# PaddlePaddle/Parakeet

Hardware: NVIDIA H100
Metric: audio-samples/sec (higher is better)
Workload: dtype bf16x3 (split-bf16 operands, fp32 accumulate; fp32-grade, 1e-3 parity)

## Files before the change

### parakeet_b200/csrc/pk_common.cu

```cuda
#include <stdarg.h>
#include <stdio.h>
#include <string.h>

#include <atomic>

#include "pk_host.h"

namespace pk {

static thread_local char g_err[512] = "";
static std::atomic<long long> g_launches{0};

void set_error(const char* fmt, ...) {
  va_list ap;
  va_start(ap, fmt);
  vsnprintf(g_err, sizeof(g_err), fmt, ap);
  va_end(ap);
}

int fail(int code, const char* fmt, ...) {
  va_list ap;
  va_start(ap, fmt);
  vsnprintf(g_err, sizeof(g_err), fmt, ap);
  va_end(ap);
  return code;
}

void count_launch(int n) { g_launches.fetch_add(n, std::memory_order_relaxed); }

int sm_count() {
  static std::atomic<int> cache[64];
  int dev = 0;
  if (cudaGetDevice(&dev) != cudaSuccess || dev < 0 || dev >= 64) return 132;
  int n = cache[dev].load(std::memory_order_relaxed);
  if (n == 0) {
    if (cudaDeviceGetAttribute(&n, cudaDevAttrMultiProcessorCount, dev) != cudaSuccess || n <= 0) n = 132;
    cache[dev].store(n, std::memory_order_relaxed);
  }
  return n;
}

typedef CUresult (*EncodeTiledFn)(CUtensorMap*, CUtensorMapDataType, cuuint32_t, void*, const cuuint64_t*, const cuuint64_t*,
                                  const cuuint32_t*, const cuuint32_t*, CUtensorMapInterleave, CUtensorMapSwizzle,
                                  CUtensorMapL2promotion, CUtensorMapFloatOOBfill);

static EncodeTiledFn get_encode_fn() {
  static EncodeTiledFn fn = nullptr;
  if (fn == nullptr) {
    void* p = nullptr;
    cudaDriverEntryPointQueryResult qres;
    if (cudaGetDriverEntryPoint("cuTensorMapEncodeTiled", &p, cudaEnableDefault, &qres) == cudaSuccess &&
        qres == cudaDriverEntryPointSuccess)
      fn = reinterpret_cast<EncodeTiledFn>(p);
  }
  return fn;
}

int encode_tmap_bf16_3d(CUtensorMap* out, const void* base, uint64_t cols, uint64_t rows, uint64_t batches,
                        uint64_t row_stride_elems, uint64_t batch_stride_elems, uint32_t box_rows) {
  EncodeTiledFn fn = get_encode_fn();
  if (fn == nullptr) return fail(PK_ERR_CUDA, "cuTensorMapEncodeTiled entry point not available (no CUDA driver?)");
  if (batches == 0) batches = 1;
  if (batch_stride_elems == 0) batch_stride_elems = row_stride_elems * rows;
  cuuint64_t dims[3] = {cols, rows, batches};
  cuuint64_t strides[2] = {row_stride_elems * 2, batch_stride_elems * 2};
  cuuint32_t box[3] = {64, box_rows, 1};
  cuuint32_t estr[3] = {1, 1, 1};
  if ((strides[0] & 15) || (strides[1] & 15)) return fail(PK_ERR_INVALID_ARG, "TMA strides must be multiples of 16 bytes");
  CUresult r = fn(out, CU_TENSOR_MAP_DATA_TYPE_BFLOAT16, 3, const_cast<void*>(base), dims, strides, box, estr,
                  CU_TENSOR_MAP_INTERLEAVE_NONE, CU_TENSOR_MAP_SWIZZLE_128B, CU_TENSOR_MAP_L2_PROMOTION_L2_256B,
                  CU_TENSOR_MAP_FLOAT_OOB_FILL_NONE);
  if (r != CUDA_SUCCESS)
    return fail(PK_ERR_CUDA, "cuTensorMapEncodeTiled failed (%d): cols=%llu rows=%llu batches=%llu ld=%llu bs=%llu box_rows=%u",
                static_cast<int>(r), (unsigned long long)cols, (unsigned long long)rows, (unsigned long long)batches,
                (unsigned long long)row_stride_elems, (unsigned long long)batch_stride_elems, box_rows);
  return PK_OK;
}

int encode_tmap_bf16_planes(CUtensorMap* out, const void* hi, const void* lo, uint64_t cols, uint64_t rows, uint64_t batches,
                            uint64_t row_stride_elems, uint64_t batch_stride_elems, uint32_t box_rows, uint32_t box_cols) {
  EncodeTiledFn fn = get_encode_fn();
  if (fn == nullptr) return fail(PK_ERR_CUDA, "cuTensorMapEncodeTiled entry point not available (no CUDA driver?)");
  if (box_cols != 64 && box_cols != 16) return fail(PK_ERR_INVALID_ARG, "box_cols must be 64 or 16 (got %u)", box_cols);
  const CUtensorMapSwizzle swz = box_cols == 64 ? CU_TENSOR_MAP_SWIZZLE_128B : CU_TENSOR_MAP_SWIZZLE_32B;
  const long long plane = static_cast<const char*>(lo) - static_cast<const char*>(hi);
  if (plane <= 0 || (plane & 15) || plane >= (1ll << 40))
    return fail(PK_ERR_INVALID_ARG, "split planes must come from one allocation, lo after hi at a 16-byte multiple (ops.Split.empty / zeros)");
  if (batches == 0) batches = 1;
  if (batch_stride_elems == 0) batch_stride_elems = row_stride_elems * rows;
  cuuint64_t dims[4] = {cols, rows, batches, 2};
  cuuint64_t strides[3] = {row_stride_elems * 2, batch_stride_elems * 2, static_cast<cuuint64_t>(plane)};
  cuuint32_t box[4] = {box_cols, box_rows, 1, 2};
  cuuint32_t estr[4] = {1, 1, 1, 1};
  if ((strides[0] & 15) || (strides[1] & 15)) return fail(PK_ERR_INVALID_ARG, "TMA strides must be multiples of 16 bytes");
  CUresult r = fn(out, CU_TENSOR_MAP_DATA_TYPE_BFLOAT16, 4, const_cast<void*>(hi), dims, strides, box, estr,
                  CU_TENSOR_MAP_INTERLEAVE_NONE, swz, CU_TENSOR_MAP_L2_PROMOTION_L2_256B,
                  CU_TENSOR_MAP_FLOAT_OOB_FILL_NONE);
  if (r != CUDA_SUCCESS)
    return fail(PK_ERR_CUDA, "cuTensorMapEncodeTiled (4-D planes) failed (%d): cols=%llu rows=%llu batches=%llu ld=%llu bs=%llu plane=%lld",
                static_cast<int>(r), (unsigned long long)cols, (unsigned long long)rows, (unsigned long long)batches,
                (unsigned long long)row_stride_elems, (unsigned long long)batch_stride_elems, plane);
  return PK_OK;
}

}

extern "C" int pk_version(void) { return 100;  }
extern "C" const char* pk_last_error(void) { return pk::g_err; }
extern "C" int64_t pk_launch_count(void) { return pk::g_launches.load(std::memory_order_relaxed); }
```

### parakeet_b200/csrc/pk_host.h

```cpp
#pragma once
#include <cuda.h>
#include <cuda_runtime.h>
#include <stdint.h>

#include "../../include/parakeet_b200.h"

namespace pk {

void set_error(const char* fmt, ...);
int fail(int code, const char* fmt, ...);

#define PK_CHECK_ARG(cond, ...)                                   \
  do {                                                            \
    if (!(cond)) return ::pk::fail(PK_ERR_INVALID_ARG, __VA_ARGS__); \
  } while (0)

#define PK_CHECK_CUDA(expr)                                                                          \
  do {                                                                                               \
    cudaError_t _e = (expr);                                                                         \
    if (_e != cudaSuccess) return ::pk::fail(PK_ERR_CUDA, "%s: %s", #expr, cudaGetErrorString(_e)); \
  } while (0)

int encode_tmap_bf16_3d(CUtensorMap* out, const void* base, uint64_t cols, uint64_t rows, uint64_t batches,
                        uint64_t row_stride_elems, uint64_t batch_stride_elems, uint32_t box_rows);

int encode_tmap_bf16_planes(CUtensorMap* out, const void* hi, const void* lo, uint64_t cols, uint64_t rows, uint64_t batches,
                            uint64_t row_stride_elems, uint64_t batch_stride_elems, uint32_t box_rows, uint32_t box_cols = 64);

int sm_count();
void count_launch(int n = 1);

}
```

### parakeet_b200/csrc/pk_sm90.cuh

```cuda
#pragma once
#include <cuda.h>
#include <cuda_bf16.h>
#include <cuda_runtime.h>
#include <stdint.h>

namespace pk {

constexpr int kSwizzleBytes = 128;
constexpr int kChunkK = 64;

__device__ __forceinline__ uint32_t smem_u32(const void* p) {
  return static_cast<uint32_t>(__cvta_generic_to_shared(p));
}

__device__ __forceinline__ void fence_barrier_init() {
  asm volatile("fence.mbarrier_init.release.cluster;" ::: "memory");
}

__device__ __forceinline__ void fence_proxy_async_all() { asm volatile("fence.proxy.async;" ::: "memory"); }
__device__ __forceinline__ void fence_proxy_async_shared() { asm volatile("fence.proxy.async.shared::cta;" ::: "memory"); }

__device__ __forceinline__ void tma_prefetch_desc(const CUtensorMap* tm) {
  asm volatile("prefetch.tensormap [%0];" ::"l"(reinterpret_cast<uint64_t>(tm)) : "memory");
}

constexpr int kWgmmaK = 16;

__device__ __forceinline__ uint64_t make_smem_desc_sw128(uint32_t smem_addr) {
  uint64_t d = 0;
  d |= static_cast<uint64_t>((smem_addr & 0x3FFFFu) >> 4);
  d |= static_cast<uint64_t>(1) << 16;
  d |= static_cast<uint64_t>(1024 >> 4) << 32;
  d |= static_cast<uint64_t>(1) << 62;
  return d;
}
__device__ __forceinline__ uint64_t desc_kstep(int k) { return static_cast<uint64_t>((k * kWgmmaK * 2) >> 4); }
__device__ __forceinline__ uint64_t make_smem_desc_sw32(uint32_t smem_addr) {
  uint64_t d = 0;
  d |= static_cast<uint64_t>((smem_addr & 0x3FFFFu) >> 4);
  d |= static_cast<uint64_t>(1) << 16;
  d |= static_cast<uint64_t>(256 >> 4) << 32;
  d |= static_cast<uint64_t>(3) << 62;
  return d;
}

__device__ __forceinline__ void wgmma_fence() { asm volatile("wgmma.fence.sync.aligned;" ::: "memory"); }
__device__ __forceinline__ void wgmma_commit() { asm volatile("wgmma.commit_group.sync.aligned;" ::: "memory"); }
template <int N>
__device__ __forceinline__ void wgmma_wait() { asm volatile("wgmma.wait_group.sync.aligned %0;" ::"n"(N) : "memory"); }
template <int R>
__device__ __forceinline__ void reg_fence(float (&d)[R]) {
#pragma unroll
  for (int i = 0; i < R; ++i) asm volatile("" : "+f"(d[i])::"memory");
}
template <uint32_t kRegs>
__device__ __forceinline__ void setmaxnreg_dec() { asm volatile("setmaxnreg.dec.sync.aligned.u32 %0;" ::"n"(kRegs)); }
template <uint32_t kRegs>
__device__ __forceinline__ void setmaxnreg_inc() { asm volatile("setmaxnreg.inc.sync.aligned.u32 %0;" ::"n"(kRegs)); }
__device__ __forceinline__ void named_bar_sync(int id, int threads) {
  asm volatile("bar.sync %0, %1;" ::"r"(id), "r"(threads) : "memory");
}
__device__ __forceinline__ void named_bar_arrive(int id, int threads) {
  asm volatile("bar.arrive %0, %1;" ::"r"(id), "r"(threads) : "memory");
}

#define PK_F8(i) "+f"(d[i]), "+f"(d[i + 1]), "+f"(d[i + 2]), "+f"(d[i + 3]), "+f"(d[i + 4]), "+f"(d[i + 5]), "+f"(d[i + 6]), "+f"(d[i + 7])
#define PK_F32(i) PK_F8(i), PK_F8(i + 8), PK_F8(i + 16), PK_F8(i + 24)
#define PK_D32 "%0,%1,%2,%3,%4,%5,%6,%7,%8,%9,%10,%11,%12,%13,%14,%15,%16,%17,%18,%19,%20,%21,%22,%23,%24,%25,%26,%27,%28,%29,%30,%31"
#define PK_D64 PK_D32 ",%32,%33,%34,%35,%36,%37,%38,%39,%40,%41,%42,%43,%44,%45,%46,%47,%48,%49,%50,%51,%52,%53,%54,%55,%56,%57,%58,%59,%60,%61,%62,%63"
#define PK_D96 PK_D64 ",%64,%65,%66,%67,%68,%69,%70,%71,%72,%73,%74,%75,%76,%77,%78,%79,%80,%81,%82,%83,%84,%85,%86,%87,%88,%89,%90,%91,%92,%93,%94,%95"
#define PK_D128 PK_D96 ",%96,%97,%98,%99,%100,%101,%102,%103,%104,%105,%106,%107,%108,%109,%110,%111,%112,%113,%114,%115,%116,%117,%118,%119,%120,%121,%122,%123,%124,%125,%126,%127"
__device__ __forceinline__ void wgmma_ss_n64(float (&d)[32], uint64_t adesc, uint64_t bdesc, uint32_t accumulate) {
  asm volatile("{\n.reg .pred p;\nsetp.ne.b32 p, %34, 0;\n"
               "wgmma.mma_async.sync.aligned.m64n64k16.f32.bf16.bf16 {" PK_D32 "}, %32, %33, p, 1, 1, 0, 0;\n}\n"
               : PK_F32(0) : "l"(adesc), "l"(bdesc), "r"(accumulate));
}
__device__ __forceinline__ void wgmma_ss_n128(float (&d)[64], uint64_t adesc, uint64_t bdesc, uint32_t accumulate) {
  asm volatile("{\n.reg .pred p;\nsetp.ne.b32 p, %66, 0;\n"
               "wgmma.mma_async.sync.aligned.m64n128k16.f32.bf16.bf16 {" PK_D64 "}, %64, %65, p, 1, 1, 0, 0;\n}\n"
               : PK_F32(0), PK_F32(32) : "l"(adesc), "l"(bdesc), "r"(accumulate));
}
__device__ __forceinline__ void wgmma_ss_n256(float (&d)[128], uint64_t adesc, uint64_t bdesc, uint32_t accumulate) {
  asm volatile("{\n.reg .pred p;\nsetp.ne.b32 p, %130, 0;\n"
               "wgmma.mma_async.sync.aligned.m64n256k16.f32.bf16.bf16 {" PK_D128 "}, %128, %129, p, 1, 1, 0, 0;\n}\n"
               : PK_F32(0), PK_F32(32), PK_F32(64), PK_F32(96) : "l"(adesc), "l"(bdesc), "r"(accumulate));
}
__device__ __forceinline__ void wgmma_rs_n64(float (&d)[32], const uint32_t (&a)[4], uint64_t bdesc, uint32_t accumulate) {
  asm volatile("{\n.reg .pred p;\nsetp.ne.b32 p, %37, 0;\n"
               "wgmma.mma_async.sync.aligned.m64n64k16.f32.bf16.bf16 {" PK_D32 "}, {%32,%33,%34,%35}, %36, p, 1, 1, 0;\n}\n"
               : PK_F32(0) : "r"(a[0]), "r"(a[1]), "r"(a[2]), "r"(a[3]), "l"(bdesc), "r"(accumulate));
}
__device__ __forceinline__ void wgmma_rs_n128(float (&d)[64], const uint32_t (&a)[4], uint64_t bdesc, uint32_t accumulate) {
  asm volatile("{\n.reg .pred p;\nsetp.ne.b32 p, %69, 0;\n"
               "wgmma.mma_async.sync.aligned.m64n128k16.f32.bf16.bf16 {" PK_D64 "}, {%64,%65,%66,%67}, %68, p, 1, 1, 0;\n}\n"
               : PK_F32(0), PK_F32(32) : "r"(a[0]), "r"(a[1]), "r"(a[2]), "r"(a[3]), "l"(bdesc), "r"(accumulate));
}
__device__ __forceinline__ void wgmma_rs_n192(float (&d)[96], const uint32_t (&a)[4], uint64_t bdesc, uint32_t accumulate) {
  asm volatile("{\n.reg .pred p;\nsetp.ne.b32 p, %101, 0;\n"
               "wgmma.mma_async.sync.aligned.m64n192k16.f32.bf16.bf16 {" PK_D96 "}, {%96,%97,%98,%99}, %100, p, 1, 1, 0;\n}\n"
               : PK_F32(0), PK_F32(32), PK_F32(64) : "r"(a[0]), "r"(a[1]), "r"(a[2]), "r"(a[3]), "l"(bdesc), "r"(accumulate));
}
#undef PK_F32
#undef PK_F8

__device__ __forceinline__ void philox4x32_10(uint32_t c0, uint32_t c1, uint32_t c2, uint32_t c3, uint32_t k0, uint32_t k1, uint32_t* out) {
#pragma unroll
  for (int r = 0; r < 10; ++r) {
    const uint32_t hi0 = __umulhi(0xD2511F53u, c0), lo0 = 0xD2511F53u * c0;
    const uint32_t hi1 = __umulhi(0xCD9E8D57u, c2), lo1 = 0xCD9E8D57u * c2;
    c0 = hi1 ^ c1 ^ k0; c1 = lo1; c2 = hi0 ^ c3 ^ k1; c3 = lo0;
    k0 += 0x9E3779B9u; k1 += 0xBB67AE85u;
  }
  out[0] = c0; out[1] = c1; out[2] = c2; out[3] = c3;
}

__device__ __forceinline__ void split_bf16(float v, __nv_bfloat16& hi, __nv_bfloat16& lo) {
  hi = __float2bfloat16_rn(v);
  lo = __float2bfloat16_rn(v - __bfloat162float(hi));
}
__device__ __forceinline__ uint32_t pack_bf16x2(__nv_bfloat16 a, __nv_bfloat16 b) {
  return static_cast<uint32_t>(__bfloat16_as_ushort(a)) | (static_cast<uint32_t>(__bfloat16_as_ushort(b)) << 16);
}
__device__ __forceinline__ void split8(const float* v, uint4& hi, uint4& lo) {
  __nv_bfloat16 h[8], l[8];
#pragma unroll
  for (int i = 0; i < 8; ++i) split_bf16(v[i], h[i], l[i]);
  hi = make_uint4(pack_bf16x2(h[0], h[1]), pack_bf16x2(h[2], h[3]), pack_bf16x2(h[4], h[5]), pack_bf16x2(h[6], h[7]));
  lo = make_uint4(pack_bf16x2(l[0], l[1]), pack_bf16x2(l[2], l[3]), pack_bf16x2(l[4], l[5]), pack_bf16x2(l[6], l[7]));
}


__device__ __forceinline__ float4 lds_f4(uint32_t addr) {
  float4 v;
  asm volatile("ld.shared.v4.f32 {%0, %1, %2, %3}, [%4];" : "=f"(v.x), "=f"(v.y), "=f"(v.z), "=f"(v.w) : "r"(addr));
  return v;
}
__device__ __forceinline__ uint32_t lds_u32(uint32_t addr) {
  uint32_t v;
  asm volatile("ld.shared.u32 %0, [%1];" : "=r"(v) : "r"(addr) : "memory");
  return v;
}
__device__ __forceinline__ void sts_u32(uint32_t addr, uint32_t v) {
  asm volatile("st.shared.u32 [%0], %1;" ::"r"(addr), "r"(v) : "memory");
}

__device__ __forceinline__ void mbar_init_a(uint32_t bar, uint32_t count) {
  asm volatile("mbarrier.init.shared::cta.b64 [%0], %1;" ::"r"(bar), "r"(count) : "memory");
}
__device__ __forceinline__ void mbar_arrive_expect_tx_a(uint32_t bar, uint32_t bytes) {
  asm volatile("mbarrier.arrive.expect_tx.shared::cta.b64 _, [%0], %1;" ::"r"(bar), "r"(bytes) : "memory");
}
__device__ __forceinline__ void mbar_arrive_a(uint32_t bar) {
  asm volatile("mbarrier.arrive.shared::cta.b64 _, [%0];" ::"r"(bar) : "memory");
}
__device__ __forceinline__ void mbar_wait_a(uint32_t bar, uint32_t parity) {
  uint32_t ok = 0;
  for (uint32_t spin = 0; spin < (1u << 26); ++spin) {
    asm volatile(
        "{\n"
        ".reg .pred p;\n"
        "mbarrier.try_wait.parity.shared::cta.b64 p, [%1], %2;\n"
        "selp.u32 %0, 1, 0, p;\n"
        "}\n"
        : "=r"(ok)
        : "r"(bar), "r"(parity)
        : "memory");
    if (ok) return;
  }
  __trap();
}
__device__ __forceinline__ void tma_load_3d_a(uint32_t smem_dst, const CUtensorMap* tm, uint32_t bar, int c0, int c1, int c2) {
  asm volatile(
      "cp.async.bulk.tensor.3d.shared::cluster.global.tile.mbarrier::complete_tx::bytes [%0], [%1, {%3, %4, %5}], [%2];"
      ::"r"(smem_dst), "l"(reinterpret_cast<uint64_t>(tm)), "r"(bar), "r"(c0), "r"(c1), "r"(c2)
      : "memory");
}
__device__ __forceinline__ void tma_load_4d_a(uint32_t smem_dst, const CUtensorMap* tm, uint32_t bar, int c0, int c1, int c2, int c3) {
  asm volatile(
      "cp.async.bulk.tensor.4d.shared::cluster.global.tile.mbarrier::complete_tx::bytes [%0], [%1, {%3, %4, %5, %6}], [%2];"
      ::"r"(smem_dst), "l"(reinterpret_cast<uint64_t>(tm)), "r"(bar), "r"(c0), "r"(c1), "r"(c2), "r"(c3)
      : "memory");
}
__device__ __forceinline__ void tma_store_4d_a(const CUtensorMap* tm, uint32_t smem_src, int c0, int c1, int c2, int c3) {
  asm volatile("cp.async.bulk.tensor.4d.global.shared::cta.bulk_group [%0, {%2, %3, %4, %5}], [%1];"
               ::"l"(reinterpret_cast<uint64_t>(tm)), "r"(smem_src), "r"(c0), "r"(c1), "r"(c2), "r"(c3)
               : "memory");
}
__device__ __forceinline__ void bulk_prefetch_l2(const void* gptr, uint32_t bytes) {
  asm volatile("cp.async.bulk.prefetch.L2.global [%0], %1;" ::"l"(reinterpret_cast<uint64_t>(gptr)), "r"(bytes) : "memory");
}
__device__ __forceinline__ void bulk_commit() { asm volatile("cp.async.bulk.commit_group;" ::: "memory"); }
template <int N>
__device__ __forceinline__ void bulk_wait_read() { asm volatile("cp.async.bulk.wait_group.read %0;" ::"n"(N) : "memory"); }


constexpr int kStageSlotBytes = 64 * 32 * 4;
__device__ __forceinline__ uint32_t stage_addr(uint32_t slot, int row, int col) {
  return slot + row * 128 + ((((col >> 2) ^ (row & 7)) << 4) | ((col & 3) << 2));
}
template <int R>
__device__ __forceinline__ void stage_store(uint32_t slot, const float (&d)[R], int C, int wg_thread) {
  const int w = wg_thread >> 5, lane = wg_thread & 31;
  const int r0 = 16 * w + (lane >> 2), c0 = 2 * (lane & 3);
#pragma unroll
  for (int jj = 0; jj < 4; ++jj) {
    const int j = 4 * C + jj;
    asm volatile("st.shared.v2.f32 [%0], {%1, %2};" ::"r"(stage_addr(slot, r0, 8 * jj + c0)), "f"(d[4 * j]), "f"(d[4 * j + 1]) : "memory");
    asm volatile("st.shared.v2.f32 [%0], {%1, %2};" ::"r"(stage_addr(slot, r0 + 8, 8 * jj + c0)), "f"(d[4 * j + 2]), "f"(d[4 * j + 3])
                 : "memory");
  }
}
__device__ __forceinline__ void stage_load_row(uint32_t slot, int row, float (&v)[32]) {
#pragma unroll
  for (int k = 0; k < 8; ++k) {
    const float4 x = lds_f4(slot + row * 128 + ((k ^ (row & 7)) << 4));
    v[4 * k] = x.x; v[4 * k + 1] = x.y; v[4 * k + 2] = x.z; v[4 * k + 3] = x.w;
  }
}

}
```

### parakeet_b200/csrc/pwg_fc.cu

```cuda
#include <stdlib.h>
#include <string.h>

#include <algorithm>

#include "pk_host.h"
#include "pk_sm90.cuh"

namespace pk {
namespace fc {

constexpr int kPwgR = 64;
constexpr int kPwgG = 128;
constexpr int kATile = 128 * kSwizzleBytes;
constexpr int kQTile = 64 * kSwizzleBytes;
constexpr int kConsumerThreads = 256;
constexpr int kThreads = kConsumerThreads + 128;
constexpr int kFcG1Chunks = 4;
constexpr int kFcStages = 6;
constexpr int kFcStageBytes = 2 * kQTile;
constexpr int kFcUBytes = 2 * 64 * 32;
constexpr int kFcPBytes = 2 * 128 * 32;
constexpr int kFcW1Bytes = 3 * 2 * kATile;
constexpr int kFcW2Bytes = 2 * kATile;
constexpr int kFcSmem = kFcW1Bytes + kFcW2Bytes + kFcStages * kFcStageBytes + 1024 + 256;
static_assert(kFcUBytes + kFcPBytes <= kFcStageBytes, "the conditioning operands share one ring stage");
static_assert(kFcSmem <= 227 * 1024, "shared memory budget");

struct FcLayerArgs {
  int batch, t, dil, hop;
  int u_period, u_start_row, u_end_base;
  int p_row0;
  const int32_t* lens;
  float gate_c[128];
  float out_b[64];
  float k_a, k_g;
  float* skip;
  int skip_init;
};

__device__ __forceinline__ float ex2_approx(float x) {
  float y;
  asm("ex2.approx.ftz.f32 %0, %1;" : "=f"(y) : "f"(x));
  return y;
}
__device__ __forceinline__ float rcp_approx(float x) {
  float y;
  asm("rcp.approx.ftz.f32 %0, %1;" : "=f"(y) : "f"(x));
  return y;
}
__device__ __forceinline__ void split2(float a, float b, uint32_t& hi, uint32_t& lo) {
  const __nv_bfloat162 h = __floats2bfloat162_rn(a, b);
  hi = *reinterpret_cast<const uint32_t*>(&h);
  const float ra = a - __uint_as_float(hi << 16);
  const float rb = b - __uint_as_float(hi & 0xffff0000u);
  const __nv_bfloat162 l = __floats2bfloat162_rn(ra, rb);
  lo = *reinterpret_cast<const uint32_t*>(&l);
}

struct FcTileIter {
  int idx, step, tiles_per_b, total, t;
  const int32_t* lens;
  __device__ FcTileIter(const FcLayerArgs& p)
      : idx(static_cast<int>(blockIdx.x) - static_cast<int>(gridDim.x)), step(gridDim.x),
        tiles_per_b((p.t + 255) >> 8), total(((p.t + 255) >> 8) * p.batch * 2), t(p.t), lens(p.lens) {}
  __device__ bool next(int& b, int& m0, int& half) {
    for (;;) {
      idx += step;
      if (idx >= total) return false;
      const int w = idx >> 1;
      half = idx & 1;
      b = w / tiles_per_b;
      m0 = (w % tiles_per_b) * 256;
      const int len = lens ? min(__ldg(lens + b), t) : t;
      if (m0 < len) return true;
    }
  }
};

__global__ void __launch_bounds__(kThreads, 1)
pwg_layer_fc_kernel(const __grid_constant__ CUtensorMap tm_x, const __grid_constant__ CUtensorMap tm_u,
                    const __grid_constant__ CUtensorMap tm_p,
                    const __grid_constant__ CUtensorMap tm_w1_hi, const __grid_constant__ CUtensorMap tm_w1_lo,
                    const __grid_constant__ CUtensorMap tm_w2_hi, const __grid_constant__ CUtensorMap tm_w2_lo,
                    const __grid_constant__ CUtensorMap tm_y, const FcLayerArgs p) {
  extern __shared__ uint8_t smem_raw[];
  const uint32_t smem = (smem_u32(smem_raw) + 1023u) & ~1023u;
  const uint32_t w1 = smem;
  const uint32_t w2 = w1 + kFcW1Bytes;
  const uint32_t ring = w2 + kFcW2Bytes;
  const uint32_t bars = ring + kFcStages * kFcStageBytes;
  const uint32_t full_bar = bars;
  const uint32_t empty_bar = full_bar + 8 * kFcStages;
  const uint32_t w_bar = empty_bar + 8 * kFcStages;

  const int warp = threadIdx.x >> 5;
  const int lane = threadIdx.x & 31;

  if (threadIdx.x == kConsumerThreads) {
    tma_prefetch_desc(&tm_x); tma_prefetch_desc(&tm_u); tma_prefetch_desc(&tm_p);
    tma_prefetch_desc(&tm_w1_hi); tma_prefetch_desc(&tm_w1_lo); tma_prefetch_desc(&tm_w2_hi); tma_prefetch_desc(&tm_w2_lo);
    tma_prefetch_desc(&tm_y);
    for (int s = 0; s < kFcStages; ++s) { mbar_init_a(full_bar + 8 * s, 1); mbar_init_a(empty_bar + 8 * s, 4); }
    mbar_init_a(w_bar, 1);
    fence_barrier_init();
  }
  __syncthreads();

  if (warp >= kConsumerThreads / 32) {
    setmaxnreg_dec<40>();
    if (warp == kConsumerThreads / 32 && lane == 0) {
      mbar_arrive_expect_tx_a(w_bar, kFcW1Bytes + kFcW2Bytes);
      for (int j = 0; j < 3; ++j) {
        tma_load_3d_a(w1 + j * 2 * kATile, &tm_w1_hi, w_bar, j * kChunkK, 0, 0);
        tma_load_3d_a(w1 + j * 2 * kATile + kATile, &tm_w1_lo, w_bar, j * kChunkK, 0, 0);
      }
      tma_load_3d_a(w2, &tm_w2_hi, w_bar, 0, 0, 0);
      tma_load_3d_a(w2 + kATile, &tm_w2_lo, w_bar, 0, 0, 0);
      uint32_t it = 0;
      FcTileIter ti(p);
      int b, m0, half;
      while (ti.next(b, m0, half)) {
        const int mh = m0 + 128 * half;
        const int len = p.lens ? min(__ldg(p.lens + b), p.t) : p.t;
        const int m1 = ((len - 128) >> 7) << 7;
        const int urow = mh == 0 ? p.u_start_row
                         : (mh + 128 > len - 128) ? p.u_end_base + 384 * b + min(mh - m1, 256)
                                                  : mh % p.u_period;
        const int j0 = (m0 / p.hop - 2) & ~7;
        for (int wg = 0; wg < 2; ++wg) {
          const int rows = min(64, p.t - (mh + 64 * wg));
          if (!p.skip_init && rows > 0)
            bulk_prefetch_l2(p.skip + (static_cast<long long>(b) * p.t + mh + 64 * wg) * 64, rows * 64 * 4);
          for (int j = 0; j < kFcG1Chunks; ++j, ++it) {
            const int s = it % kFcStages;
            mbar_wait_a(empty_bar + 8 * s, ((it / kFcStages) & 1) ^ 1);
            const uint32_t st = ring + s * kFcStageBytes;
            const uint32_t fb = full_bar + 8 * s;
            if (j == 2) {
              mbar_arrive_expect_tx_a(fb, kFcUBytes + kFcPBytes);
              tma_load_4d_a(st, &tm_u, fb, 0, urow + 64 * wg, 0, 0);
              tma_load_4d_a(st + kFcUBytes, &tm_p, fb, j0, p.p_row0, b, 0);
            } else {
              mbar_arrive_expect_tx_a(fb, kFcStageBytes);
              const int wj = j == 0 ? 0 : j == 1 ? 2 : 1;
              tma_load_4d_a(st, &tm_x, fb, 0, mh + 64 * wg + (wj - 1) * p.dil, b, 0);
            }
          }
        }
      }
    }
  } else {
    setmaxnreg_inc<232>();
    const int wg = warp >> 2;
    const int rl = 16 * (warp & 3) + (lane >> 2);
    const int cq = 2 * (lane & 3);
    const float kSqrtHalf = 0.70710678118654752440f;
    mbar_wait_a(w_bar, 0);
    uint32_t it = wg * kFcG1Chunks;
    FcTileIter ti(p);
    int b, m0, half;
    bool more = ti.next(b, m0, half);
    bool first = true;
    while (more) {
      const int mh = m0 + 128 * half;
      float acc1[64], acc2[64];
      if (wg == 1 || !first) named_bar_sync(1 + wg, kConsumerThreads);
      first = false;
#pragma unroll
      for (int j = 0; j < kFcG1Chunks; ++j) {
        const int s = (it + j) % kFcStages;
        mbar_wait_a(full_bar + 8 * s, ((it + j) / kFcStages) & 1);
        const uint32_t st = ring + s * kFcStageBytes;
        wgmma_fence();
        if (j == 2) {
          const uint64_t a_hi = make_smem_desc_sw32(st), a_lo = make_smem_desc_sw32(st + kFcUBytes / 2);
          const uint64_t b_hi = make_smem_desc_sw32(st + kFcUBytes), b_lo = make_smem_desc_sw32(st + kFcUBytes + kFcPBytes / 2);
          wgmma_ss_n128(acc1, a_hi, b_hi, 1);
          wgmma_ss_n128(acc1, a_lo, b_hi, 1);
          wgmma_ss_n128(acc1, a_hi, b_lo, 1);
        } else {
          const int wj = j == 0 ? 0 : j == 1 ? 2 : 1;
          const uint64_t a_hi = make_smem_desc_sw128(st), a_lo = make_smem_desc_sw128(st + kQTile);
          const uint64_t b_hi = make_smem_desc_sw128(w1 + wj * 2 * kATile), b_lo = make_smem_desc_sw128(w1 + wj * 2 * kATile + kATile);
#pragma unroll
          for (int k = 0; k < 4; ++k) {
            wgmma_ss_n128(acc1, a_hi + desc_kstep(k), b_hi + desc_kstep(k), !(j == 0 && k == 0));
            wgmma_ss_n128(acc1, a_lo + desc_kstep(k), b_hi + desc_kstep(k), 1);
            wgmma_ss_n128(acc1, a_hi + desc_kstep(k), b_lo + desc_kstep(k), 1);
          }
        }
        wgmma_commit();
        if (j == kFcG1Chunks - 1) {
#pragma unroll
          for (int jj = 0; jj < 8; ++jj) {
#pragma unroll
            for (int hh = 0; hh < 2; ++hh) {
              const int r = rl + 8 * hh;
              const uint32_t off = r * kSwizzleBytes + ((((8 * jj + cq) >> 3) ^ (r & 7)) << 4) + (cq & 7) * 2;
              const uint32_t xh = lds_u32(st + off), xl = lds_u32(st + kQTile + off);
              acc2[4 * jj + 2 * hh] = 0.f;
              acc2[4 * jj + 2 * hh + 1] = 0.f;
              acc2[32 + 4 * jj + 2 * hh] = __uint_as_float(xh << 16) + __uint_as_float(xl << 16);
              acc2[32 + 4 * jj + 2 * hh + 1] = __uint_as_float(xh & 0xffff0000u) + __uint_as_float(xl & 0xffff0000u);
            }
          }
        }
        if (j > 0) {
          wgmma_wait<1>();
          __syncwarp();
          if (lane == 0) mbar_arrive_a(empty_bar + 8 * ((it + j - 1) % kFcStages));
        }
      }
      wgmma_wait<0>();
      reg_fence(acc1);
      const int cs = (it + kFcG1Chunks - 1) % kFcStages;
      const uint32_t ystage = ring + cs * kFcStageBytes;
      it += 2 * kFcG1Chunks;
      int nb, nm0, nhalf;
      const bool next = ti.next(nb, nm0, nhalf);
      if (wg == 0 || next) named_bar_arrive(2 - wg, kConsumerThreads);
      uint32_t zh[16], zl[16];
#pragma unroll
      for (int jj = 0; jj < 8; ++jj) {
        float z[4];
#pragma unroll
        for (int e = 0; e < 4; ++e) {
          const int c = 8 * jj + cq + (e & 1);
          const float e1 = ex2_approx(fminf(fmaf(acc1[4 * jj + e], p.k_a, p.gate_c[c]), 60.f));
          const float e2 = ex2_approx(fmaf(acc1[32 + 4 * jj + e], p.k_g, p.gate_c[64 + c]));
          const float t1 = 1.f + e1;
          z[e] = (1.f - e1) * rcp_approx(fmaf(t1, e2, t1));
        }
        split2(z[0], z[1], zh[2 * jj], zl[2 * jj]);
        split2(z[2], z[3], zh[2 * jj + 1], zl[2 * jj + 1]);
      }
      const uint64_t b2_hi = make_smem_desc_sw128(w2), b2_lo = make_smem_desc_sw128(w2 + kATile);
      wgmma_fence();
#pragma unroll
      for (int k = 0; k < 4; ++k) {
        const uint32_t ah[4] = {zh[4 * k], zh[4 * k + 1], zh[4 * k + 2], zh[4 * k + 3]};
        const uint32_t al[4] = {zl[4 * k], zl[4 * k + 1], zl[4 * k + 2], zl[4 * k + 3]};
        wgmma_rs_n128(acc2, ah, b2_hi + desc_kstep(k), 1);
        wgmma_rs_n128(acc2, al, b2_hi + desc_kstep(k), 1);
        wgmma_rs_n128(acc2, ah, b2_lo + desc_kstep(k), 1);
      }
      wgmma_commit();
      wgmma_wait<0>();
      reg_fence(acc2);
      const int len = p.lens ? min(__ldg(p.lens + b), p.t) : p.t;
#pragma unroll
      for (int hh = 0; hh < 2; ++hh) {
        const int r = rl + 8 * hh;
        const bool live = mh + wg * 64 + r < len;
#pragma unroll
        for (int jj = 0; jj < 8; ++jj) {
          const int c = 8 * jj + cq;
          const float y0 = live ? (acc2[32 + 4 * jj + 2 * hh] + p.out_b[c]) * kSqrtHalf : 0.f;
          const float y1 = live ? (acc2[32 + 4 * jj + 2 * hh + 1] + p.out_b[c + 1]) * kSqrtHalf : 0.f;
          uint32_t oh, ol;
          split2(y0, y1, oh, ol);
          const uint32_t off = r * kSwizzleBytes + (((c >> 3) ^ (r & 7)) << 4) + (cq & 7) * 2;
          sts_u32(ystage + off, oh);
          sts_u32(ystage + kQTile + off, ol);
        }
      }
      fence_proxy_async_shared();
      named_bar_sync(3 + wg, 128);
      const bool store_lane = (threadIdx.x & 127) == 0;
      if (store_lane) {
        tma_store_4d_a(&tm_y, ystage, 0, mh + wg * 64, b, 0);
        bulk_commit();
      }
#pragma unroll
      for (int hh = 0; hh < 2; ++hh) {
        const int trow = mh + wg * 64 + rl + 8 * hh;
        if (trow < p.t) {
          const long long row_off = (static_cast<long long>(b) * p.t + trow) * 64;
#pragma unroll
          for (int jj = 0; jj < 8; ++jj) {
            float* d2 = p.skip + row_off + 8 * jj + cq;
            const float s0 = acc2[4 * jj + 2 * hh], s1 = acc2[4 * jj + 2 * hh + 1];
            if (p.skip_init) *reinterpret_cast<float2*>(d2) = make_float2(s0, s1);
            else asm volatile("red.global.add.v2.f32 [%0], {%1, %2};" ::"l"(d2), "f"(s0), "f"(s1) : "memory");
          }
        }
      }
      if (store_lane) {
        bulk_wait_read<0>();
#pragma unroll
        for (int w = 0; w < 4; ++w) mbar_arrive_a(empty_bar + 8 * cs);
      }
      b = nb; m0 = nm0; half = nhalf; more = next;
    }
  }
}

}
}

extern "C" int pk_pwg_residual_layer_fc(const pk_pwg_layer_fc_args* a, pk_stream_t stream) {
  using namespace pk;
  using namespace pk::fc;
  PK_CHECK_ARG(a != nullptr, "args is NULL");
  PK_CHECK_ARG(a->batch > 0 && a->t > 0 && a->dilation >= 1 && a->hop >= 256, "bad batch/t/dilation/hop (hop must be >= 256)");
  PK_CHECK_ARG(a->x_hi && a->x_lo && a->y_hi && a->y_lo && a->u_hi && a->u_lo && a->p_hi && a->p_lo && a->w1_hi && a->w1_lo &&
               a->w2_hi && a->w2_lo && a->bias1 && a->bias2 && a->skip, "NULL pointer in pk_pwg_layer_fc_args");
  PK_CHECK_ARG(a->x_hi != a->y_hi, "layer output must not alias its input");
  PK_CHECK_ARG(a->u_period > 0 && (a->u_period % 128) == 0 && a->u_start_row >= a->u_period && a->u_end_base >= a->u_start_row + 128 &&
               a->u_rows >= a->u_end_base + 384 * a->batch, "bad compact band table layout");
  PK_CHECK_ARG(a->p_rows > 0 && a->p_row0 >= 0 && a->p_row0 + 128 <= a->p_rows && (a->p_ld % 8) == 0 && a->p_ld >= 64 && a->p_frames > 0 &&
               a->p_frames <= a->p_ld, "bad P plane geometry");
  CUtensorMap tx, tu, tp, tw1_hi, tw1_lo, tw2_hi, tw2_lo, ty;
  int rc;
  const uint64_t T = a->t, B = a->batch;
  if ((rc = encode_tmap_bf16_planes(&tx, a->x_hi, a->x_lo, kPwgR, T, B, kPwgR, T * kPwgR, 64))) return rc;
  if ((rc = encode_tmap_bf16_planes(&ty, a->y_hi, a->y_lo, kPwgR, T, B, kPwgR, T * kPwgR, 64))) return rc;
  if ((rc = encode_tmap_bf16_planes(&tu, a->u_hi, a->u_lo, 64, a->u_rows, 1, 64, 0, 64, 16))) return rc;
  const uint64_t prow = a->p_rows, pld = a->p_ld;
  if ((rc = encode_tmap_bf16_planes(&tp, a->p_hi, a->p_lo, pld, prow, B, pld, prow * pld, 128, 16))) return rc;
  const uint64_t k1 = 5 * kChunkK;
  if ((rc = encode_tmap_bf16_3d(&tw1_hi, a->w1_hi, 3 * kChunkK, kPwgG, 1, k1, k1 * kPwgG, 128))) return rc;
  if ((rc = encode_tmap_bf16_3d(&tw1_lo, a->w1_lo, 3 * kChunkK, kPwgG, 1, k1, k1 * kPwgG, 128))) return rc;
  if ((rc = encode_tmap_bf16_3d(&tw2_hi, a->w2_hi, 64, 128, 1, 64, 0, 128))) return rc;
  if ((rc = encode_tmap_bf16_3d(&tw2_lo, a->w2_lo, 64, 128, 1, 64, 0, 128))) return rc;
  static bool attr_set = false;
  if (!attr_set) {
    PK_CHECK_CUDA(cudaFuncSetAttribute(pwg_layer_fc_kernel, cudaFuncAttributeMaxDynamicSharedMemorySize, kFcSmem));
    attr_set = true;
  }
  FcLayerArgs p;
  p.batch = a->batch; p.t = a->t; p.dil = a->dilation; p.hop = a->hop;
  p.u_period = a->u_period; p.u_start_row = a->u_start_row; p.u_end_base = a->u_end_base;
  p.p_row0 = a->p_row0;
  p.lens = a->lens; p.skip = a->skip; p.skip_init = a->skip_init;
  constexpr float kLog2e = 1.4426950408889634f;
  p.k_a = -2.f * kLog2e; p.k_g = -kLog2e;
  for (int i = 0; i < 64; ++i) {
    p.gate_c[i] = -2.f * kLog2e * a->bias1[i];
    p.gate_c[64 + i] = -kLog2e * a->bias1[64 + i];
    p.out_b[i] = a->bias2[64 + i];
  }
  const cudaStream_t st = static_cast<cudaStream_t>(stream);
  const int tiles = ((a->t + 255) / 256) * 2 * a->batch;
  const int grid = std::min(tiles, sm_count());
  pwg_layer_fc_kernel<<<grid, kThreads, kFcSmem, static_cast<cudaStream_t>(stream)>>>(tx, tu, tp, tw1_hi, tw1_lo, tw2_hi, tw2_lo, ty, p);
  PK_CHECK_CUDA(cudaGetLastError());
  count_launch();
  return PK_OK;
}
```

Measured before the change: 68.22 million.

## Write skip accumulator via TMA reduce-add from dedicated smem staging

Replaces the per-thread global red.add/stores of the fp32 skip accumulator with a swizzled shared-memory staging buffer and a TMA bulk reduce-add (or plain store on init). The y output also gets its own staging area instead of reusing a ring stage, so the ring stage is released right after GEMM1. A pair of ping-pong barriers now serializes the two consumer warpgroups on the staging buffers. To fit the extra shared memory the ring depth drops from six stages to four, and the L2 prefetch of skip is removed, which may reduce load latency hiding.

```diff
diff --git a/parakeet_b200/csrc/pk_common.cu b/parakeet_b200/csrc/pk_common.cu
--- a/parakeet_b200/csrc/pk_common.cu
+++ b/parakeet_b200/csrc/pk_common.cu
@@ -77,6 +77,27 @@
   return PK_OK;
 }
 
+int encode_tmap_f32_3d(CUtensorMap* out, const void* base, uint64_t rows, uint64_t batches, uint64_t batch_stride_elems,
+                       uint32_t box_rows) {
+  EncodeTiledFn fn = get_encode_fn();
+  if (fn == nullptr) return fail(PK_ERR_CUDA, "cuTensorMapEncodeTiled entry point not available (no CUDA driver?)");
+  if (batches == 0) batches = 1;
+  if (batch_stride_elems == 0) batch_stride_elems = 32 * rows;
+  cuuint64_t dims[3] = {32, rows, batches};
+  cuuint64_t strides[2] = {32 * 4, batch_stride_elems * 4};
+  cuuint32_t box[3] = {32, box_rows, 1};
+  cuuint32_t estr[3] = {1, 1, 1};
+  if (strides[1] & 15) return fail(PK_ERR_INVALID_ARG, "TMA strides must be multiples of 16 bytes");
+  CUresult r = fn(out, CU_TENSOR_MAP_DATA_TYPE_FLOAT32, 3, const_cast<void*>(base), dims, strides, box, estr,
+                  CU_TENSOR_MAP_INTERLEAVE_NONE, CU_TENSOR_MAP_SWIZZLE_128B, CU_TENSOR_MAP_L2_PROMOTION_L2_256B,
+                  CU_TENSOR_MAP_FLOAT_OOB_FILL_NONE);
+  if (r != CUDA_SUCCESS)
+    return fail(PK_ERR_CUDA, "cuTensorMapEncodeTiled (fp32) failed (%d): rows=%llu batches=%llu bs=%llu box_rows=%u",
+                static_cast<int>(r), (unsigned long long)rows, (unsigned long long)batches, (unsigned long long)batch_stride_elems,
+                box_rows);
+  return PK_OK;
+}
+
 int encode_tmap_bf16_planes(CUtensorMap* out, const void* hi, const void* lo, uint64_t cols, uint64_t rows, uint64_t batches,
                             uint64_t row_stride_elems, uint64_t batch_stride_elems, uint32_t box_rows, uint32_t box_cols) {
   EncodeTiledFn fn = get_encode_fn();
diff --git a/parakeet_b200/csrc/pk_host.h b/parakeet_b200/csrc/pk_host.h
--- a/parakeet_b200/csrc/pk_host.h
+++ b/parakeet_b200/csrc/pk_host.h
@@ -27,6 +27,9 @@
 int encode_tmap_bf16_planes(CUtensorMap* out, const void* hi, const void* lo, uint64_t cols, uint64_t rows, uint64_t batches,
                             uint64_t row_stride_elems, uint64_t batch_stride_elems, uint32_t box_rows, uint32_t box_cols = 64);
 
+int encode_tmap_f32_3d(CUtensorMap* out, const void* base, uint64_t rows, uint64_t batches, uint64_t batch_stride_elems,
+                       uint32_t box_rows);
+
 int sm_count();
 void count_launch(int n = 1);
 
diff --git a/parakeet_b200/csrc/pk_sm90.cuh b/parakeet_b200/csrc/pk_sm90.cuh
--- a/parakeet_b200/csrc/pk_sm90.cuh
+++ b/parakeet_b200/csrc/pk_sm90.cuh
@@ -142,6 +142,9 @@
 }
 __device__ __forceinline__ void sts_u32(uint32_t addr, uint32_t v) {
   asm volatile("st.shared.u32 [%0], %1;" ::"r"(addr), "r"(v) : "memory");
+}
+__device__ __forceinline__ void sts_f2(uint32_t addr, float a, float b) {
+  asm volatile("st.shared.v2.f32 [%0], {%1, %2};" ::"r"(addr), "f"(a), "f"(b) : "memory");
 }
 
 __device__ __forceinline__ void mbar_init_a(uint32_t bar, uint32_t count) {
@@ -186,8 +189,15 @@
                ::"l"(reinterpret_cast<uint64_t>(tm)), "r"(smem_src), "r"(c0), "r"(c1), "r"(c2), "r"(c3)
                : "memory");
 }
-__device__ __forceinline__ void bulk_prefetch_l2(const void* gptr, uint32_t bytes) {
-  asm volatile("cp.async.bulk.prefetch.L2.global [%0], %1;" ::"l"(reinterpret_cast<uint64_t>(gptr)), "r"(bytes) : "memory");
+__device__ __forceinline__ void tma_store_3d_a(const CUtensorMap* tm, uint32_t smem_src, int c0, int c1, int c2) {
+  asm volatile("cp.async.bulk.tensor.3d.global.shared::cta.bulk_group [%0, {%2, %3, %4}], [%1];"
+               ::"l"(reinterpret_cast<uint64_t>(tm)), "r"(smem_src), "r"(c0), "r"(c1), "r"(c2)
+               : "memory");
+}
+__device__ __forceinline__ void tma_reduce_add_3d_a(const CUtensorMap* tm, uint32_t smem_src, int c0, int c1, int c2) {
+  asm volatile("cp.reduce.async.bulk.tensor.3d.global.shared::cta.add.tile.bulk_group [%0, {%2, %3, %4}], [%1];"
+               ::"l"(reinterpret_cast<uint64_t>(tm)), "r"(smem_src), "r"(c0), "r"(c1), "r"(c2)
+               : "memory");
 }
 __device__ __forceinline__ void bulk_commit() { asm volatile("cp.async.bulk.commit_group;" ::: "memory"); }
 template <int N>
diff --git a/parakeet_b200/csrc/pwg_fc.cu b/parakeet_b200/csrc/pwg_fc.cu
--- a/parakeet_b200/csrc/pwg_fc.cu
+++ b/parakeet_b200/csrc/pwg_fc.cu
@@ -16,13 +16,15 @@
 constexpr int kConsumerThreads = 256;
 constexpr int kThreads = kConsumerThreads + 128;
 constexpr int kFcG1Chunks = 4;
-constexpr int kFcStages = 6;
+constexpr int kFcStages = 4;
 constexpr int kFcStageBytes = 2 * kQTile;
 constexpr int kFcUBytes = 2 * 64 * 32;
 constexpr int kFcPBytes = 2 * 128 * 32;
 constexpr int kFcW1Bytes = 3 * 2 * kATile;
 constexpr int kFcW2Bytes = 2 * kATile;
-constexpr int kFcSmem = kFcW1Bytes + kFcW2Bytes + kFcStages * kFcStageBytes + 1024 + 256;
+constexpr int kFcYBytes = 2 * kQTile;
+constexpr int kFcSkipBytes = 64 * 64 * 4;
+constexpr int kFcSmem = kFcW1Bytes + kFcW2Bytes + kFcStages * kFcStageBytes + kFcYBytes + kFcSkipBytes + 1024 + 256;
 static_assert(kFcUBytes + kFcPBytes <= kFcStageBytes, "the conditioning operands share one ring stage");
 static_assert(kFcSmem <= 227 * 1024, "shared memory budget");
 
@@ -82,16 +84,20 @@
                     const __grid_constant__ CUtensorMap tm_p,
                     const __grid_constant__ CUtensorMap tm_w1_hi, const __grid_constant__ CUtensorMap tm_w1_lo,
                     const __grid_constant__ CUtensorMap tm_w2_hi, const __grid_constant__ CUtensorMap tm_w2_lo,
-                    const __grid_constant__ CUtensorMap tm_y, const FcLayerArgs p) {
+                    const __grid_constant__ CUtensorMap tm_y, const __grid_constant__ CUtensorMap tm_skip,
+                    const FcLayerArgs p) {
   extern __shared__ uint8_t smem_raw[];
   const uint32_t smem = (smem_u32(smem_raw) + 1023u) & ~1023u;
   const uint32_t w1 = smem;
   const uint32_t w2 = w1 + kFcW1Bytes;
   const uint32_t ring = w2 + kFcW2Bytes;
-  const uint32_t bars = ring + kFcStages * kFcStageBytes;
+  const uint32_t ystage = ring + kFcStages * kFcStageBytes;
+  const uint32_t sstage = ystage + kFcYBytes;
+  const uint32_t bars = sstage + kFcSkipBytes;
   const uint32_t full_bar = bars;
   const uint32_t empty_bar = full_bar + 8 * kFcStages;
   const uint32_t w_bar = empty_bar + 8 * kFcStages;
+  const uint32_t free_bar = w_bar + 8;
 
   const int warp = threadIdx.x >> 5;
   const int lane = threadIdx.x & 31;
@@ -99,9 +105,10 @@
   if (threadIdx.x == kConsumerThreads) {
     tma_prefetch_desc(&tm_x); tma_prefetch_desc(&tm_u); tma_prefetch_desc(&tm_p);
     tma_prefetch_desc(&tm_w1_hi); tma_prefetch_desc(&tm_w1_lo); tma_prefetch_desc(&tm_w2_hi); tma_prefetch_desc(&tm_w2_lo);
-    tma_prefetch_desc(&tm_y);
+    tma_prefetch_desc(&tm_y); tma_prefetch_desc(&tm_skip);
     for (int s = 0; s < kFcStages; ++s) { mbar_init_a(full_bar + 8 * s, 1); mbar_init_a(empty_bar + 8 * s, 4); }
     mbar_init_a(w_bar, 1);
+    mbar_init_a(free_bar, 1); mbar_init_a(free_bar + 8, 1);
     fence_barrier_init();
   }
   __syncthreads();
@@ -128,9 +135,6 @@
                                                   : mh % p.u_period;
         const int j0 = (m0 / p.hop - 2) & ~7;
         for (int wg = 0; wg < 2; ++wg) {
-          const int rows = min(64, p.t - (mh + 64 * wg));
-          if (!p.skip_init && rows > 0)
-            bulk_prefetch_l2(p.skip + (static_cast<long long>(b) * p.t + mh + 64 * wg) * 64, rows * 64 * 4);
           for (int j = 0; j < kFcG1Chunks; ++j, ++it) {
             const int s = it % kFcStages;
             mbar_wait_a(empty_bar + 8 * s, ((it / kFcStages) & 1) ^ 1);
@@ -161,6 +165,7 @@
     int b, m0, half;
     bool more = ti.next(b, m0, half);
     bool first = true;
+    uint32_t free_phase = wg ^ 1;
     while (more) {
       const int mh = m0 + 128 * half;
       float acc1[64], acc2[64];
@@ -213,8 +218,8 @@
       }
       wgmma_wait<0>();
       reg_fence(acc1);
-      const int cs = (it + kFcG1Chunks - 1) % kFcStages;
-      const uint32_t ystage = ring + cs * kFcStageBytes;
+      __syncwarp();
+      if (lane == 0) mbar_arrive_a(empty_bar + 8 * ((it + kFcG1Chunks - 1) % kFcStages));
       it += 2 * kFcG1Chunks;
       int nb, nm0, nhalf;
       const bool next = ti.next(nb, nm0, nhalf);
@@ -247,6 +252,8 @@
       wgmma_commit();
       wgmma_wait<0>();
       reg_fence(acc2);
+      mbar_wait_a(free_bar + 8 * wg, free_phase);
+      free_phase ^= 1;
       const int len = p.lens ? min(__ldg(p.lens + b), p.t) : p.t;
 #pragma unroll
       for (int hh = 0; hh < 2; ++hh) {
@@ -262,33 +269,20 @@
           const uint32_t off = r * kSwizzleBytes + (((c >> 3) ^ (r & 7)) << 4) + (cq & 7) * 2;
           sts_u32(ystage + off, oh);
           sts_u32(ystage + kQTile + off, ol);
+          const int line = 2 * r + (c >> 5);
+          sts_f2(sstage + line * 128 + ((((c & 31) >> 2) ^ (line & 7)) << 4) + (c & 3) * 4, acc2[4 * jj + 2 * hh],
+                 acc2[4 * jj + 2 * hh + 1]);
         }
       }
       fence_proxy_async_shared();
       named_bar_sync(3 + wg, 128);
-      const bool store_lane = (threadIdx.x & 127) == 0;
-      if (store_lane) {
+      if ((threadIdx.x & 127) == 0) {
         tma_store_4d_a(&tm_y, ystage, 0, mh + wg * 64, b, 0);
+        if (p.skip_init) tma_store_3d_a(&tm_skip, sstage, 0, 2 * (mh + wg * 64), b);
+        else tma_reduce_add_3d_a(&tm_skip, sstage, 0, 2 * (mh + wg * 64), b);
         bulk_commit();
-      }
-#pragma unroll
-      for (int hh = 0; hh < 2; ++hh) {
-        const int trow = mh + wg * 64 + rl + 8 * hh;
-        if (trow < p.t) {
-          const long long row_off = (static_cast<long long>(b) * p.t + trow) * 64;
-#pragma unroll
-          for (int jj = 0; jj < 8; ++jj) {
-            float* d2 = p.skip + row_off + 8 * jj + cq;
-            const float s0 = acc2[4 * jj + 2 * hh], s1 = acc2[4 * jj + 2 * hh + 1];
-            if (p.skip_init) *reinterpret_cast<float2*>(d2) = make_float2(s0, s1);
-            else asm volatile("red.global.add.v2.f32 [%0], {%1, %2};" ::"l"(d2), "f"(s0), "f"(s1) : "memory");
-          }
-        }
-      }
-      if (store_lane) {
         bulk_wait_read<0>();
-#pragma unroll
-        for (int w = 0; w < 4; ++w) mbar_arrive_a(empty_bar + 8 * cs);
+        mbar_arrive_a(free_bar + 8 * (wg ^ 1));
       }
       b = nb; m0 = nm0; half = nhalf; more = next;
     }
@@ -310,11 +304,12 @@
                a->u_rows >= a->u_end_base + 384 * a->batch, "bad compact band table layout");
   PK_CHECK_ARG(a->p_rows > 0 && a->p_row0 >= 0 && a->p_row0 + 128 <= a->p_rows && (a->p_ld % 8) == 0 && a->p_ld >= 64 && a->p_frames > 0 &&
                a->p_frames <= a->p_ld, "bad P plane geometry");
-  CUtensorMap tx, tu, tp, tw1_hi, tw1_lo, tw2_hi, tw2_lo, ty;
+  CUtensorMap tx, tu, tp, tw1_hi, tw1_lo, tw2_hi, tw2_lo, ty, ts;
   int rc;
   const uint64_t T = a->t, B = a->batch;
   if ((rc = encode_tmap_bf16_planes(&tx, a->x_hi, a->x_lo, kPwgR, T, B, kPwgR, T * kPwgR, 64))) return rc;
   if ((rc = encode_tmap_bf16_planes(&ty, a->y_hi, a->y_lo, kPwgR, T, B, kPwgR, T * kPwgR, 64))) return rc;
+  if ((rc = encode_tmap_f32_3d(&ts, a->skip, 2 * T, B, 0, 128))) return rc;
   if ((rc = encode_tmap_bf16_planes(&tu, a->u_hi, a->u_lo, 64, a->u_rows, 1, 64, 0, 64, 16))) return rc;
   const uint64_t prow = a->p_rows, pld = a->p_ld;
   if ((rc = encode_tmap_bf16_planes(&tp, a->p_hi, a->p_lo, pld, prow, B, pld, prow * pld, 128, 16))) return rc;
@@ -343,7 +338,7 @@
   const cudaStream_t st = static_cast<cudaStream_t>(stream);
   const int tiles = ((a->t + 255) / 256) * 2 * a->batch;
   const int grid = std::min(tiles, sm_count());
-  pwg_layer_fc_kernel<<<grid, kThreads, kFcSmem, static_cast<cudaStream_t>(stream)>>>(tx, tu, tp, tw1_hi, tw1_lo, tw2_hi, tw2_lo, ty, p);
+  pwg_layer_fc_kernel<<<grid, kThreads, kFcSmem, static_cast<cudaStream_t>(stream)>>>(tx, tu, tp, tw1_hi, tw1_lo, tw2_hi, tw2_lo, ty, ts, p);
   PK_CHECK_CUDA(cudaGetLastError());
   count_launch();
   return PK_OK;
```

Result: faster. 73.07 million, median of 6 (+7.1%).
